# coqui-ai/TTS

Measured on NVIDIA H100. Metric: audio_samples_per_sec, higher is better.
Workload: dtype f32

## Files before the change

### tts_b200/csrc/common.cuh

```cuda
#pragma once
#include <cuda_runtime.h>
#include <stdint.h>
#include <stdio.h>
#include <atomic>
#include <mutex>
#include <string>
#include <vector>

namespace b200tts {

void set_error(const char* fmt, ...);
const char* last_error();

#define B200_CUDA_OK(expr)                                                                  \
    do {                                                                                    \
        cudaError_t _e = (expr);                                                            \
        if (_e != cudaSuccess) {                                                            \
            ::b200tts::set_error("%s:%d: %s -> %s", __FILE__, __LINE__, #expr,              \
                                 cudaGetErrorString(_e));                                   \
            return 2;                                                                       \
        }                                                                                   \
    } while (0)

#define B200_REQUIRE(cond, ...)                                                             \
// ... 53 lines not shown
};

struct ConvIO {
    const float* x = nullptr; long long x_bs = 0; int x_cs = 0; int Tin = 0;
    const float* xmask = nullptr; long long xmask_bs = 0;
    float in_slope = 1.0f;
    const float* cond = nullptr; long long cond_bs = 0;
    float* y = nullptr; long long y_bs = 0; int y_cs = 0; int Tout = 0;
    const float* res = nullptr; long long res_bs = 0; int res_cs = 0;
    const float* ymask = nullptr; long long ymask_bs = 0;
    float* y2 = nullptr; long long y2_bs = 0; int y2_cs = 0;
    int split = 0;
    float scale = 1.0f;
    float post_div = 1.0f;
    int act = ACT_NONE;
    float act_param = 0.f;
    int flags = 0;
    int B = 1;
    unsigned* peak_bits = nullptr;
    const int* lens = nullptr; int rate_out = 1, need_out = 0, rate_in = 1, need_in = 0;
    int q_lo = 0, q_hi = 0x7fffffff, in_lo = 0, in_hi = 0x7fffffff;
    int reflect = 0;
    int near_src = 0;
    const float* film = nullptr; long long film_bs = 0; int film_cs = 0; int film_half = 0;
    const float* act_add = nullptr;
};

int pack_conv(ConvLayer& L, const float* w, const float* bias, int Cout, int Cin, int K, int dil, int pad,
              int gate_half = 0, const int* in_perm = nullptr, const int* out_perm = nullptr);
int pack_conv_transpose(ConvLayer& L, const float* w, const float* bias, int Cin, int Cout, int Kt, int stride,
                        int padding, int output_padding = 0);
void free_conv(ConvLayer& L);
int launch_conv(const ConvLayer& L, const ConvIO& io, cudaStream_t stream);
int conv_tc_error_flag();
int pack_tc(void** dst, const std::vector<float>& Wl, int rows, int Cin, int K, int prec, int G, float** rscale = nullptr);
int tc_device(int** err, int* num_sms, size_t* max_smem);
enum : int { DISPATCH_FMA = 0, DISPATCH_TC3 = 3, DISPATCH_TC3_GROUPED = 5, DISPATCH_ROW1 = 6,
             DISPATCH_TC16 = 8, DISPATCH_TC16_GROUPED = 9,
             DISPATCH_ATTN_TC3 = 10, DISPATCH_ATTN_FMA = 11,
             DISPATCH_TC3W_TF32 = 12, DISPATCH_TC3W_F16X3 = 14, DISPATCH_FMA_WG = 16,
             DISPATCH_LSTM_BI = 18, DISPATCH_LSTM_CELL = 19, DISPATCH_HMM_LINEAR = 20, DISPATCH_HMM_STEP = 21,
             DISPATCH_PWGAN_TC = 22, DISPATCH_PWGAN_AUX = 23 };
void dispatch_begin();
int dispatch_end(int* ids, int cap);
void dispatch_note(int id);
inline int conv_transpose_out_len(const ConvLayer& L, int Tin) {
    return (Tin - 1) * L.ups - 2 * L.tr_pad + L.tr_kernel + L.tr_outpad;
}

template <class T> inline int upload(T** dst, const T* src, size_t n) {
    *dst = nullptr;
    if (n == 0) return 0;
    B200_CUDA_OK(cudaMalloc((void**)dst, n * sizeof(T)));
    B200_CUDA_OK(cudaMemcpy(*dst, src, n * sizeof(T), cudaMemcpyHostToDevice));
    return 0;
}

struct Arena {
    char* base; size_t cap; size_t off;
    Arena(void* p, size_t bytes) : base((char*)p), cap(bytes), off(0) {}
    float* f32(size_t n) {
        size_t bytes = (n * sizeof(float) + 255) & ~size_t(255);
        if (off + bytes > cap) return nullptr;
        float* r = (float*)(base + off);
        off += bytes;
        return r;
// ... 6 lines not shown
```

### tts_b200/csrc/conv1d.cu

```cuda
#include "common.cuh"
#include "engines.cuh"
#include "conv_tc.cuh"
#include "conv_tc3.cuh"

#include <cuda_bf16.h>
#include <cuda_fp16.h>
#include <stdarg.h>
#include <string.h>

#include <algorithm>
#include <cmath>

namespace b200tts {

static thread_local char g_err[1024] = "";
unsigned long long g_launch_count = 0;

void set_error(const char* fmt, ...) {
    va_list ap;
    va_start(ap, fmt);
    vsnprintf(g_err, sizeof(g_err), fmt, ap);
    va_end(ap);
}
const char* last_error() { return g_err; }
// ... 711 lines not shown
}
static void set_ragged(tc3::Tc3Args& t, const ConvKArgs& a, size_t& smem, size_t max_smem) {
    t.lens = nullptr; t.rate_q = 1; t.need_q = 0; t.rate_in = 1; t.need_in = 0; t.pref_off = 0;
    if (!a.lens) return;
    const size_t off = (smem + 15) / 16 * 16, extra = tc3::ragged_table_bytes(t.B);
    if (off + extra > max_smem) return;
    t.lens = a.lens; t.rate_q = a.rate_out; t.need_q = a.need_out; t.rate_in = a.rate_in; t.need_in = a.need_in;
    t.pref_off = (int)off;
    smem = off + extra;
}
static void set_window(tc3::Tc3Args& t, const ConvKArgs& a) {
    t.Tin = std::min(a.Tin, a.in_hi);
    t.q_lo = a.q_lo; t.q_hi = a.q_hi; t.in_lo = a.in_lo; t.t_lo = a.q_lo / t.tstep;
    const int hi = std::min(a.Tq, a.q_hi);
    t.n_ttiles = std::max(0, (hi + t.tstep - 1) / t.tstep - t.t_lo);
}

static int tc_device_init(int d) {
    int smem_optin = 0;
    B200_CUDA_OK(cudaDeviceGetAttribute(&smem_optin, cudaDevAttrMaxSharedMemoryPerBlockOptin, d));
    for (int p : {tc::PREC_FP32, tc::PREC_BF16, tc::PREC_FP16, tc::PREC_F16X3}) {
        for (bool lean : {true, false})
            B200_CUDA_OK(cudaFuncSetAttribute(tc3::plain_kernel(p, lean), cudaFuncAttributeMaxDynamicSharedMemorySize, smem_optin));
        B200_CUDA_OK(cudaFuncSetAttribute(tc3::plain_kernel(p, true, true), cudaFuncAttributeMaxDynamicSharedMemorySize, smem_optin));
        for (int g : {2, 4})
            for (bool refl : {false, true})
                B200_CUDA_OK(cudaFuncSetAttribute(tc3::grouped_kernel(g, p, refl), cudaFuncAttributeMaxDynamicSharedMemorySize,
                                                  smem_optin));
        for (bool near : {false, true})
            if (tc3::wavegrad_kernel(p, near))
                B200_CUDA_OK(cudaFuncSetAttribute(tc3::wavegrad_kernel(p, near), cudaFuncAttributeMaxDynamicSharedMemorySize,
                                                  smem_optin));
    }
    int* flag = nullptr;
    B200_CUDA_OK(cudaHostAlloc((void**)&flag, 2 * sizeof(int), cudaHostAllocMapped | cudaHostAllocPortable));
    flag[0] = flag[tc::ERR_RANGE] = 0;
    g_tc_dev[d].err = flag;
    g_tc_dev[d].max_smem = smem_optin;
    B200_CUDA_OK(cudaDeviceGetAttribute(&g_tc_dev[d].num_sms, cudaDevAttrMultiProcessorCount, d));
    return 0;
}

int tc_device(int** err, int* num_sms, size_t* max_smem) {
    int dev = 0;
    if (int rc = device_once(g_tc_once, &dev, tc_device_init)) return rc;
    int* const g_tc_err = g_tc_dev[dev].err;
    B200_REQUIRE(*reinterpret_cast<volatile int*>(g_tc_err) == 0,
                 "tensor-core conv: an earlier launch on device %d hit a pipeline timeout (its output is invalid)", dev);
    volatile int* const range_err = reinterpret_cast<volatile int*>(g_tc_err + tc::ERR_RANGE);
    if (*range_err) {
        *range_err = 0;
        B200_REQUIRE(false, "tensor-core conv: an earlier split-fp16 launch on device %d read an activation with |x| >= 65504, "
                            "outside fp16's range (its output is invalid; B200TTS_PRECISION_TF32X3 takes such models)", dev);
    }
    *err = g_tc_err;
    if (num_sms) *num_sms = g_tc_dev[dev].num_sms;
    if (max_smem) *max_smem = (size_t)g_tc_dev[dev].max_smem;
    return 0;
}

static int try_launch_tc(const ConvLayer& L, const ConvIO& io, const ConvKArgs& a, cudaStream_t st) {
    if (L.tc_prec == TC_NONE || a.Tq < 128) return -1;
    if (a.act == ACT_LOGCLAMP || a.act == ACT_TANH) return -1;
    if (!(a.in_slope >= 0.f && a.in_slope <= 1.f)) return -1;
    const bool needs_v3 = (a.flags & (EPI_MASK_PRE | EPI_SPLIT | EPI_ACCUM2 | EPI_GATE)) != 0;
    int* g_tc_err = nullptr;
// ... 25 lines not shown
    t.mask_pre = (a.flags & EPI_MASK_PRE) ? 1 : 0;
    t.gate = (a.flags & EPI_GATE) ? 1 : 0;
    t.split = (a.flags & EPI_SPLIT) ? a.split : 0;
    t.y2 = a.y2; t.y2_bs = a.y2_bs; t.y2_cs = a.y2_cs; t.accum2 = (a.flags & EPI_ACCUM2) ? 1 : 0;
    t.rows_pad = rows_pad; t.raw_w = rows_pad + 4;
    t.B = io.B; t.n_rtiles = (L.Rows + tc3::MROWS - 1) / tc3::MROWS;
    set_window(t, a);
    t.err = g_tc_err;
    size_t smem = tc3::smem_bytes3(rows_pad, L.tc_prec);
    set_ragged(t, a, smem, max_smem);
    const bool plain_epi = L.ups == 1 && !t.gate && t.split == 0 && !t.relu && !t.ymask && t.scale == 1.f && t.post_div == 1.f;
    const bool reflect = a.reflect != 0;
    if (reflect && !grouped && !plain_epi) return -1;
    if (wg) {
        t.near_src = a.near_src; t.near_scale = a.near_scale;
        t.film = a.film; t.film_bs = a.film_bs; t.film_cs = a.film_cs; t.film_half = a.film_half;
        t.act_add = a.act_add; t.lrelu = a.act == ACT_LRELU; t.act_param = a.act_param;
    }
    const tc3::Tc3Kernel k = wg ? tc3::wavegrad_kernel(L.tc_prec, a.near_src > 0)
                                : grouped ? tc3::grouped_kernel(G, L.tc_prec, reflect) : tc3::plain_kernel(L.tc_prec, plain_epi, reflect);
    const long long tiles = (long long)t.B * t.n_ttiles * t.n_rtiles;
    const int grid = (int)std::max(1LL, tiles < num_sms ? tiles : num_sms);
    B200_CUDA_OK(launch_tc3(k, grid, smem, st, t));
    count_launch();
    const bool b16 = L.tc_prec == tc::PREC_BF16 || L.tc_prec == tc::PREC_FP16;
    if (wg)
        dispatch_note((L.tc_prec == tc::PREC_F16X3 ? DISPATCH_TC3W_F16X3 : DISPATCH_TC3W_TF32) + (a.near_src > 0 ? 1 : 0));
    else
        dispatch_note(grouped ? (b16 ? DISPATCH_TC16_GROUPED : DISPATCH_TC3_GROUPED) : (b16 ? DISPATCH_TC16 : DISPATCH_TC3));
    B200_CUDA_OK(cudaGetLastError());
    return 0;
}

int conv_tc_error_flag() {
    int f = 0;
    for (int d = 0; d < MAX_DEVICES; ++d) {
        if (!g_tc_dev[d].err) continue;
        const volatile int* e = g_tc_dev[d].err;
        if (e[0]) f |= 1;
        if (e[tc::ERR_RANGE]) f |= 2;
    }
    return f;
}

int launch_conv(const ConvLayer& L, const ConvIO& io, cudaStream_t st) {
    B200_REQUIRE(L.w && io.x && io.y, "launch_conv: null tensor");
    ConvKArgs a;
    memset(&a, 0, sizeof(a));
    a.x = io.x; a.x_bs = io.x_bs; a.x_cs = io.x_cs; a.Tin = io.Tin;
    a.xmask = io.xmask; a.xmask_bs = io.xmask_bs; a.in_slope = io.in_slope;
    a.w = L.w; a.bias = L.bias; a.cond = io.cond; a.cond_bs = io.cond_bs;
    a.Cin = L.Cin; a.CinPad = L.CinPad; a.K = L.K; a.dil = L.dil; a.pad = L.pad; a.Rows = L.Rows; a.ups = L.ups;
    a.y = io.y; a.y_bs = io.y_bs; a.y_cs = io.y_cs; a.Tout = io.Tout;
    a.Tq = (L.ups > 1) ? (io.Tout + L.ups - 1) / L.ups : io.Tout;
    a.res = io.res; a.res_bs = io.res_bs; a.res_cs = io.res_cs;
    a.ymask = io.ymask; a.ymask_bs = io.ymask_bs;
    a.y2 = io.y2; a.y2_bs = io.y2_bs; a.y2_cs = io.y2_cs; a.split = io.split;
    a.scale = io.scale; a.post_div = io.post_div; a.act = io.act; a.act_param = io.act_param; a.flags = io.flags;
    a.lens = io.lens; a.rate_out = io.rate_out; a.need_out = io.need_out; a.rate_in = io.rate_in; a.need_in = io.need_in;
    a.q_lo = std::max(0, io.q_lo); a.q_hi = io.q_hi; a.in_lo = std::max(0, io.in_lo); a.in_hi = io.in_hi;
    const bool windowed = a.q_lo > 0 || a.q_hi < a.Tq;
    a.reflect = io.reflect ? 1 : 0;
    if (a.reflect) {
        B200_REQUIRE(L.pad <= io.Tin - 1, "launch_conv: reflection padding %d needs at least %d input columns, got %d", L.pad,
                     L.pad + 1, io.Tin);
        B200_REQUIRE(!io.lens && !windowed && a.in_lo == 0 && a.in_hi == 0x7fffffff && L.ups == 1 && !io.xmask,
// ... 67 lines not shown
```

### tts_b200/csrc/conv_tc3.cuh

```cuda
#pragma once
#include <cuda_runtime.h>
#include <stdint.h>

#include "conv_tc.cuh"

namespace b200tts {
namespace tc3 {

using namespace tc;

constexpr int TT2 = 256;
constexpr int MROWS = 128;
constexpr int KC2 = 8;
constexpr int KC16 = 16;
constexpr int RAWS = 324;
constexpr int NRAW = 3;
constexpr int NA2 = 2;
constexpr int NB2 = 3;
constexpr int ACC_LD = 260;
constexpr int ACC_BYTES = MROWS * ACC_LD * 4;
constexpr int NPW = 3;
constexpr int NPROD = 32 * NPW;
constexpr int NCONS = 256;
constexpr int W_PROD = 8, W_LOAD = 8 + NPW;
constexpr int NTHREADS2 = 32 * (W_LOAD + 1);

struct Tc3Args {
    const float* x; long long x_bs; int x_cs; int Tin;
    float in_slope;
    const void* w;
    const float* rscale;
    const float* bias;
    const float* cond; long long cond_bs;
    int Cin, K, dil, pad, Rows, N;
    float* y; long long y_bs; int y_cs; int Tout;
    int ups;
    int Tq;
    const float* res; long long res_bs; int res_cs;
    const float* ymask; long long ymask_bs;
    float scale; float post_div; int relu; int accum; int mask_post;
    int mask_pre;
    int gate;
    int split;
    float* y2; long long y2_bs; int y2_cs; int accum2;
    int KJ;
    int dil_blk;
    int tstep;
    int rows_pad;
    int raw_w;
    int B, n_ttiles, n_rtiles;
    int* err;
    const int* lens; int rate_q, need_q, rate_in, need_in;
    int pref_off;
    int q_lo, q_hi, in_lo, t_lo;
    int near_src; float near_scale;
    const float* film; long long film_bs; int film_cs, film_half;
    const float* act_add; int lrelu; float act_param;
};

__device__ __forceinline__ int near_col(int t, int src, int dst, float scale) {
    if (dst == src) return t;
    if (dst == 2 * src) return t >> 1;
    return min((int)floorf(__fmul_rn((float)t, scale)), src - 1);
}

static inline size_t smem_bytes3(int rows_pad, int prec = PREC_FP32) {
    const bool b16 = prec == PREC_BF16 || prec == PREC_FP16;
    const size_t raw_ch = b16 ? KC16 : KC2, nsl = b16 ? 2 : 4;
    return (size_t)NRAW * raw_ch * RAWS * 4 + (size_t)NA2 * (nsl * rows_pad * 16) + NB2 * (nsl * MROWS * 16) + ACC_BYTES + 512;
}
static inline size_t ragged_table_bytes(int B) { return ((size_t)(B + 1) * sizeof(int) + 15) / 16 * 16; }

__device__ __forceinline__ void cp_async16(uint32_t dst, const void* src) {
    asm volatile("cp.async.cg.shared.global [%0], [%1], 16;" ::"r"(dst), "l"(src) : "memory");
}
__device__ __forceinline__ void cp_async16_zfill(uint32_t dst, const void* src, uint32_t src_bytes) {
    asm volatile("cp.async.cg.shared.global [%0], [%1], 16, %2;" ::"r"(dst), "l"(src), "r"(src_bytes) : "memory");
}
__device__ __forceinline__ void cp_async4_zfill(uint32_t dst, const void* src, uint32_t src_bytes) {
    asm volatile("cp.async.ca.shared.global [%0], [%1], 4, %2;" ::"r"(dst), "l"(src), "r"(src_bytes) : "memory");
}
__device__ __forceinline__ void named_bar_sync(int id, int n) { asm volatile("bar.sync %0, %1;" ::"r"(id), "r"(n) : "memory"); }
__device__ __forceinline__ void acc_ld16(const float* p, float* v) {
#pragma unroll
    for (int j = 0; j < 4; ++j) {
        const float4 t = *reinterpret_cast<const float4*>(p + 4 * j);
        v[4 * j] = t.x; v[4 * j + 1] = t.y; v[4 * j + 2] = t.z; v[4 * j + 3] = t.w;
    }
}

constexpr int TSTEP_GROUPED = 240;

template <bool HR, bool HA, bool SC>
__device__ __forceinline__ void lean_tile(const float* at, const float* bias, const float* rscale, const float* cond, int lane,
                                          const float* rq, float* yq, long long rcs, long long ycs, int row0, int Rows,
                                          bool do_st) {
    const int r8 = lane & 7, p4 = lane >> 3;
    const float* rrow[4];
    float* yrow[4];
    bool st_ok[4];
    float bv[4], sv[4];
#pragma unroll
    for (int i = 0; i < 4; ++i) {
        const int ri = row0 + 8 * i + r8, rci = ri < Rows ? ri : Rows - 1;
        rrow[i] = rq + (long long)rci * rcs + 4 * p4;
        yrow[i] = yq + (long long)rci * ycs + 4 * p4;
        st_ok[i] = do_st && ri < Rows;
        bv[i] = bias[rci];
        if (cond) bv[i] += __ldg(cond + rci);
        sv[i] = SC ? rscale[rci] : 1.f;
    }
    const float* ap = at + r8 * ACC_LD + 4 * p4;
    float r0[16], r1[16];
    auto pf = [&](int cg, float* r_) {
        if constexpr (HR) {
#pragma unroll
            for (int i = 0; i < 4; ++i)
                asm volatile("ld.global.v4.f32 {%0,%1,%2,%3}, [%4];" : "=f"(r_[4 * i]), "=f"(r_[4 * i + 1]), "=f"(r_[4 * i + 2]), "=f"(r_[4 * i + 3]) : "l"(rrow[i] + cg));
        }
    };
    auto group = [&](int cg, const float* rv, float* rn) {
        float o[16];
        if (cg + 16 < 128) pf(cg + 16, rn);
        if constexpr (HA) {
// ... 192 lines not shown
        if (rok) prefetch(0, rA, oA);
#pragma unroll 1
        for (int cg = 0; cg < 128; cg += 32) {
            group(cg, rA, oA, rB, oB);
            group(cg + 16, rB, oB, rA, oA);
        }
    } else {
        if (!rok) return;
        const int co = rc / ups, ph = rc - co * ups;
        float* yrow = a.y + (long long)b * a.y_bs + (long long)co * a.y_cs + ph;
        for (int cg = 0; cg < 128; cg += 16) {
            float v[16];
            acc_ld(arow + cg, v);
#pragma unroll
            for (int i = 0; i < 16; ++i) {
                const int q = qb + cg + i;
                float u = v[i] + bias;
                if (a.relu) u = fmaxf(u, 0.f);
                const long long t = (long long)q * ups;
                if (q < a.Tq && t + ph < a.Tout) yrow[t] = u;
            }
        }
    }
}

template <bool SC>
__device__ __noinline__ void general_tile_call(const Tc3Args& a_ref, const float* arow, int b, int rt, int q0, int lq, int half,
                                               int lane) {
    const Tc3Args a = a_ref;
    general_tile_body<SC>(a, arow, b, rt, q0, lq, half, lane);
}

template <int GRP, bool SC>
__device__ __forceinline__ void grouped_tile(const Tc3Args& a, const float* accs, int b, int q0, int lq, int half, int lane) {
    constexpr int CH = 128 / GRP;
    constexpr int NQ = CH / 32;
    constexpr int NV = 4 * NQ;
    const int tq = lq * 32 + lane;
    const int co = (tq * NQ) >> 2;
    const int coff = 4 * ((tq & (4 / NQ - 1)) * NQ);
    const int cbeg = half ? 128 : 0;
    const int cend = half ? a.tstep : min(128, a.tstep);
    const bool has_res = a.res != nullptr, acc_r = a.accum != 0;
    const bool vec_ok = ((a.y_cs & 3) == 0) && ((a.y_bs & 3) == 0) && ((reinterpret_cast<uintptr_t>(a.y) & 15) == 0) &&
                        (!a.res || (((a.res_cs & 3) == 0) && ((a.res_bs & 3) == 0) && ((reinterpret_cast<uintptr_t>(a.res) & 15) == 0)));
    const bool fast = vec_ok && (q0 + a.tstep <= a.Tout);
    const float* rrow = has_res ? a.res + (long long)b * a.res_bs + (long long)co * a.res_cs : nullptr;
    float* yrow = a.y + (long long)b * a.y_bs + (long long)co * a.y_cs;
    float bias = a.bias[co];
    if (a.cond) bias += __ldg(a.cond + (long long)b * a.cond_bs + co);
    const float rs = SC ? a.rscale[co] : 1.f;
    auto load = [&](const float* rr, int q, float* dst) {
#pragma unroll
        for (int j = 0; j < NQ; ++j) {
            const int qq = q + 4 * j;
            if (fast || (vec_ok && qq + 3 < a.Tout)) {
                const float4 t = *reinterpret_cast<const float4*>(rr + qq);
                dst[4 * j] = t.x; dst[4 * j + 1] = t.y; dst[4 * j + 2] = t.z; dst[4 * j + 3] = t.w;
            } else {
#pragma unroll
                for (int e = 0; e < 4; ++e) dst[4 * j + e] = rr[min(qq + e, a.Tout - 1)];
            }
        }
    };
#pragma unroll 1
    for (int cg = cbeg; cg < cend; cg += 16) {
        float R[NV], rv[NV], ov[NV];
        if (has_res) load(rrow, q0 + cg + coff, rv);
        if (acc_r) load(yrow, q0 + cg + coff, ov);
        const float* p = accs + co * ACC_LD + cg + coff;
#pragma unroll
        for (int i = 0; i < NV; ++i) {
            const float p0 = p[i], p1 = p[CH * ACC_LD + a.dil + i];
            float s = p0 + p1;
            if constexpr (GRP == 4) s += p[2 * CH * ACC_LD + 2 * a.dil + i] + p[3 * CH * ACC_LD + 3 * a.dil + i];
            if constexpr (SC) s *= rs;
            R[i] = s;
        }
#pragma unroll
        for (int i = 0; i < NV; ++i) {
            float u = R[i] + bias;
            if (a.relu) u = fmaxf(u, 0.f);
            if (has_res) u += rv[i];
            u *= a.scale;
            if (acc_r) u += ov[i];
            if (a.post_div != 1.f) u = u / a.post_div;
            R[i] = u;
        }
        const int q = q0 + cg + coff;
#pragma unroll
        for (int j = 0; j < NQ; ++j) {
            const int qq = q + 4 * j;
            if (fast || (vec_ok && qq + 3 < a.Tout)) {
                *reinterpret_cast<float4*>(yrow + qq) = make_float4(R[4 * j], R[4 * j + 1], R[4 * j + 2], R[4 * j + 3]);
            } else {
#pragma unroll
                for (int e = 0; e < 4; ++e) if (qq + e < a.Tout) yrow[qq + e] = R[4 * j + e];
            }
        }
    }
}

template <int GRP, bool LEAN = true, int PREC = PREC_FP32, bool REFL = false, bool NEAR = false, bool WG = false>
__device__ __forceinline__ void tc3_body(const Tc3Args& a) {
    extern __shared__ __align__(128) unsigned char smem[];
    constexpr bool X3 = PREC == PREC_F16X3;
    constexpr bool B16 = PREC == PREC_BF16 || PREC == PREC_FP16;
    constexpr int KCH = PREC != PREC_FP32 ? KC16 : KC2;
    constexpr int RCH = B16 ? KC16 : KC2;
    constexpr int SPC = KCH / RCH;
    constexpr int NSL = B16 ? 2 : 4;
    constexpr int SLC = PREC != PREC_FP32 ? 8 : 4;
    constexpr int NB = NB2;
    constexpr bool SC = X3;
    const int tid = threadIdx.x, warp = tid >> 5, lane = tid & 31;
    const int ROWS = a.rows_pad, RAWW = a.raw_w, K = a.KJ;
    const uint32_t rawStage = (uint32_t)RCH * RAWS * 4;
    const uint32_t slabA = (uint32_t)ROWS * 16, stageA = NSL * slabA;
    const uint32_t slabB = (uint32_t)MROWS * 16, stageB = NSL * slabB;
    unsigned char* smRaw = smem;
    unsigned char* smA = smRaw + NRAW * rawStage;
    unsigned char* smB = smA + NA2 * stageA;
    float* accs = reinterpret_cast<float*>(smB + NB * stageB);
    uint64_t* bars = reinterpret_cast<uint64_t*>(reinterpret_cast<unsigned char*>(accs) + ACC_BYTES);
    const int A_FULL = 0, A_EMPTY = NA2, B_FULL = 2 * NA2, B_EMPTY = 2 * NA2 + NB;
    const uint32_t bar0 = smem_u32(bars);
    auto BAR = [&](int i) { return bar0 + 8u * (uint32_t)i; };

    const int nchunks = (a.Cin + KCH - 1) / KCH;
    const bool ragged = a.lens != nullptr;
    int* pref = reinterpret_cast<int*>(smem + a.pref_off);
    if (ragged) {
        for (int b = tid; b < a.B; b += NTHREADS2) {
            const long long e = (long long)a.lens[b] * a.rate_q + a.need_q;
            const int ext = (int)(e < (long long)a.Tq ? (e > 0 ? e : 0) : (long long)a.Tq);
            const int t_hi = (min(ext, a.q_hi) + a.tstep - 1) / a.tstep;
// ... 197 lines not shown
                    }
                    *reinterpret_cast<uint4*>(base + i_dst[e]) = make_uint4(p[0], p[1], p[2], p[3]);
                }
            } else {
#pragma unroll
                for (int e = 0; e < MAXI; ++e) {
                    if (i_raw[e] < 0) continue;
                    float4 hi, lo;
                    float* ph = &hi.x; float* pl = &lo.x;
#pragma unroll
                    for (int i = 0; i < 4; ++i) {
                        const float w_ = fmaxf(u[e][i], u[e][i] * slope);
                        const float h = __uint_as_float(__float_as_uint(w_) & 0xFFFFE000u);
                        ph[i] = h;
                        pl[i] = w_ - h;
                    }
                    *reinterpret_cast<float4*>(base + i_dst[e]) = hi;
                    *reinterpret_cast<float4*>(base + 2 * slabA + i_dst[e]) = lo;
                }
            }
            if (++tr_ring == NRAW) tr_ring = 0;
            if (++tr_h < SPC) continue;
            tr_h = 0;
            fence_async_smem();
            __syncwarp();
            if (lane == 0) mbar_arrive(BAR(A_FULL + as));
            if (++tr_c == nchunks) { tr_c = 0; ++tr_it; tr_new = true; }
            if (++as == NA2) { as = 0; pa_empty ^= 1u; }
        }
        asm volatile("cp.async.wait_group 0;" ::: "memory");
        if (X3 && amax >= F16X3_MAX && a.err) { *reinterpret_cast<volatile int*>(a.err + ERR_RANGE) = 1; __threadfence_system(); }
    } else if (warp == W_LOAD) {
        if (lane < NB) {
            const int total = nchunks * K;
            const long long all = (long long)my_tiles * total;
            const uint32_t full = BAR(B_FULL + lane), empty = BAR(B_EMPTY + lane);
            const uint32_t dst = smem_u32(smB + lane * stageB);
            int it = 0, j = lane;
            while (j >= total && it < my_tiles) { j -= total; ++it; }
            int cur_it = -1;
            const unsigned char* wsrc = nullptr;
            uint32_t par = 1;
            bool ok = true, first = true;
            for (long long gi = lane; gi < all && ok; gi += NB) {
                if (it != cur_it) {
                    int b_, rt, q0_;
                    decode(it, b_, rt, q0_);
                    wsrc = reinterpret_cast<const unsigned char*>(a.w) + (size_t)rt * total * stageB;
                    cur_it = it;
                }
                if (!first) { ok = mbar_wait(empty, par, a.err); if (!ok) break; }
                mbar_expect_tx(full, stageB);
                bulk_g2s(dst, wsrc + (size_t)j * stageB, stageB, full);
                first = false;
                par ^= 1u;
                j += NB;
                while (j >= total) { j -= total; ++it; }
            }
        }
        __syncwarp();
    } else if (warp < W_PROD) {
        const int wg = warp >> 2, lq = warp & 3, half = warp >> 2;
        const uint64_t wdesc0 = make_desc(smem_u32(smB) + (uint32_t)wg * 64 * 16, slabB);
        const uint64_t wlo_off = (uint64_t)((2 * slabB) >> 4), wslot = (uint64_t)(stageB >> 4);
        const uint32_t whi_lds = smem_u32(smB) + (uint32_t)(lane >> 4) * slabB + (uint32_t)(warp * 16 + (lane & 15)) * 16;
        const uint64_t xstep = (uint64_t)a.dil_blk;
        bool ok = true;
        int sa = 0; uint32_t pa = 0;
        int sb = 0; uint32_t pb = 0;
        float* const st_row = accs + (wg * 64 + lq * 16 + (lane >> 2)) * ACC_LD + 2 * (lane & 3);
#pragma unroll 1
        for (int it = 0; it < my_tiles; ++it) {
            float d[128];
#pragma unroll
            for (int i = 0; i < 128; ++i) d[i] = 0.f;
            uint32_t acc = 0u;
            int rel_b = -1, rel_a = -1;
            auto release = [&]() {
                __syncwarp();
                if (lane == 0) {
                    if (rel_b >= 0) mbar_arrive(BAR(B_EMPTY + rel_b));
                    if (rel_a >= 0) mbar_arrive(BAR(A_EMPTY + rel_a));
                }
            };
#pragma unroll 1
            for (int c = 0; c < nchunks; ++c) {
// ... 10 lines not shown
                            ldsm_x4(whs, whi_lds + (uint32_t)sb * stageB);
#pragma unroll
                            for (int i = 0; i < 4; ++i) whs[i] = f16x2_times_2m11(whs[i]);
                        }
                        wgmma_fence();
                        if constexpr (PREC == PREC_BF16) {
                            wgmma_bf16_m64n256(d, w_hi, xh, acc);
                        } else if constexpr (PREC == PREC_FP16) {
                            wgmma_f16_m64n256(d, w_hi, xh, acc);
                        } else if constexpr (X3) {
                            wgmma_f16_m64n256_rs(d, whs, xl, acc);
                            wgmma_commit();
                            wgmma_f16_m64n256(d, w_lo, xh, 1u);
                            wgmma_f16_m64n256(d, w_hi, xh, 1u);
                        } else {
                            wgmma_tf32_m64n256(d, w_hi, xl, acc);
                            wgmma_tf32_m64n256(d, w_lo, xh, 1u);
                            wgmma_tf32_m64n256(d, w_hi, xh, 1u);
                        }
                        wgmma_commit();
                    }
                    wgmma_wait<1>();
                    release();
                    rel_b = sb;
                    rel_a = (k == K - 1) ? sa : -1;
                    acc = 1u;
                    xh += xstep; xl += xstep;
                    if (++sb == NB) { sb = 0; pb ^= 1u; }
                }
                if (++sa == NA2) { sa = 0; pa ^= 1u; }
            }
            wgmma_wait<0>();
            release();
            named_bar_sync(4, NCONS);
#pragma unroll
            for (int j = 0; j < 32; ++j) {
                *reinterpret_cast<float2*>(st_row + 8 * j) = make_float2(d[4 * j], d[4 * j + 1]);
                *reinterpret_cast<float2*>(st_row + 8 * ACC_LD + 8 * j) = make_float2(d[4 * j + 2], d[4 * j + 3]);
            }
            named_bar_sync(4, NCONS);
            if (!ok) continue;
            int b, rt, q0;
            decode(it, b, rt, q0);
            if constexpr (GRP > 1) {
                grouped_tile<GRP, SC>(a, accs, b, q0, lq, half, lane);
            } else {
                const int qb = q0 + half * 128;
                const float* at = accs + lq * 32 * ACC_LD + half * 128;
                const bool lean = LEAN && a.ups == 1 && !a.gate && a.split == 0 && !a.relu && !a.ymask && a.scale == 1.f &&
                                  a.post_div == 1.f && qb + 128 <= a.Tout &&
                                  ((a.y_cs & 3) == 0) && ((a.y_bs & 3) == 0) && ((reinterpret_cast<uintptr_t>(a.y) & 15) == 0) &&
                                  (!a.res || (((a.res_cs & 3) == 0) && ((a.res_bs & 3) == 0) && ((reinterpret_cast<uintptr_t>(a.res) & 15) == 0)));
                if (lean) {
                    const int row0 = rt * MROWS + lq * 32;
                    const float* cond = a.cond ? a.cond + (long long)b * a.cond_bs : nullptr;
                    float* yq = a.y + (long long)b * a.y_bs + qb;
                    const bool hres = a.res != nullptr, hacc = a.accum != 0;
                    const float* rq = hres ? a.res + (long long)b * a.res_bs + qb : yq;
                    if (hres) { if (hacc) lean_tile<true, true, SC>(at, a.bias, a.rscale, cond, lane, rq, yq, a.res_cs, a.y_cs, row0, a.Rows, true);
                                else lean_tile<true, false, SC>(at, a.bias, a.rscale, cond, lane, rq, yq, a.res_cs, a.y_cs, row0, a.Rows, true); }
                    else { if (hacc) lean_tile<false, true, SC>(at, a.bias, a.rscale, cond, lane, rq, yq, 0, a.y_cs, row0, a.Rows, true);
                           else lean_tile<false, false, SC>(at, a.bias, a.rscale, cond, lane, rq, yq, 0, a.y_cs, row0, a.Rows, true); }
                } else if constexpr (LEAN) {
                    general_tile_call<SC>(a, at + lane * ACC_LD, b, rt, q0, lq, half, lane);
                } else {
                    general_tile_body<SC, WG>(a, at + lane * ACC_LD, b, rt, q0, lq, half, lane);
                }
            }
        }
    }
}

template <int PREC, bool REFL = false>
__global__ void __launch_bounds__(NTHREADS2, 1) conv1d_tc3_kernel(const __grid_constant__ Tc3Args a) { tc3_body<1, true, PREC, REFL>(a); }
template <int PREC>
__global__ void __launch_bounds__(NTHREADS2, 1) conv1d_tc3x_kernel(const __grid_constant__ Tc3Args a) { tc3_body<1, false, PREC>(a); }
template <int GRP, int PREC, bool REFL = false>
__global__ void __launch_bounds__(NTHREADS2, 1) conv1d_tc3g_kernel(const __grid_constant__ Tc3Args a) { tc3_body<GRP, true, PREC, REFL>(a); }

template <int PREC, bool NEAR>
__global__ void __launch_bounds__(NTHREADS2, 1) conv1d_tc3w_kernel(const __grid_constant__ Tc3Args a) {
    tc3_body<1, false, PREC, false, NEAR, true>(a);
}

typedef void (*Tc3Kernel)(const Tc3Args);
static inline Tc3Kernel wavegrad_kernel(int prec, bool near) {
    if (prec == PREC_F16X3) return near ? conv1d_tc3w_kernel<PREC_F16X3, true> : conv1d_tc3w_kernel<PREC_F16X3, false>;
    if (prec == PREC_FP32) return near ? conv1d_tc3w_kernel<PREC_FP32, true> : conv1d_tc3w_kernel<PREC_FP32, false>;
    return nullptr;
}
static inline Tc3Kernel plain_kernel(int prec, bool lean, bool reflect = false) {
    if (reflect) {
        if (prec == PREC_BF16) return conv1d_tc3_kernel<PREC_BF16, true>;
        if (prec == PREC_FP16) return conv1d_tc3_kernel<PREC_FP16, true>;
        if (prec == PREC_F16X3) return conv1d_tc3_kernel<PREC_F16X3, true>;
        return conv1d_tc3_kernel<PREC_FP32, true>;
    }
    if (prec == PREC_BF16) return lean ? conv1d_tc3_kernel<PREC_BF16> : conv1d_tc3x_kernel<PREC_BF16>;
    if (prec == PREC_FP16) return lean ? conv1d_tc3_kernel<PREC_FP16> : conv1d_tc3x_kernel<PREC_FP16>;
    if (prec == PREC_F16X3) return lean ? conv1d_tc3_kernel<PREC_F16X3> : conv1d_tc3x_kernel<PREC_F16X3>;
    return lean ? conv1d_tc3_kernel<PREC_FP32> : conv1d_tc3x_kernel<PREC_FP32>;
}
template <bool REFL>
static inline Tc3Kernel grouped_kernel_t(int grp, int prec) {
    if (prec == PREC_BF16) return grp == 2 ? conv1d_tc3g_kernel<2, PREC_BF16, REFL> : conv1d_tc3g_kernel<4, PREC_BF16, REFL>;
    if (prec == PREC_FP16) return grp == 2 ? conv1d_tc3g_kernel<2, PREC_FP16, REFL> : conv1d_tc3g_kernel<4, PREC_FP16, REFL>;
    if (prec == PREC_F16X3) return grp == 2 ? conv1d_tc3g_kernel<2, PREC_F16X3, REFL> : conv1d_tc3g_kernel<4, PREC_F16X3, REFL>;
    return grp == 2 ? conv1d_tc3g_kernel<2, PREC_FP32, REFL> : conv1d_tc3g_kernel<4, PREC_FP32, REFL>;
}
static inline Tc3Kernel grouped_kernel(int grp, int prec = PREC_FP32, bool reflect = false) {
    return reflect ? grouped_kernel_t<true>(grp, prec) : grouped_kernel_t<false>(grp, prec);
// ... 5 lines not shown
```

### tts_b200/csrc/engines.cuh

```cuda
#pragma once
#include <algorithm>
#include <string.h>

#include "../../include/tts_b200.h"
#include "common.cuh"

namespace b200tts {

struct Hifigan {
    b200tts_hifigan_config c;
    ConvLayer conv_pre, cond, conv_post;
    std::vector<ConvLayer> ups;
    std::vector<std::vector<ConvLayer>> rb_c1, rb_c2;
    int prec = B200TTS_PRECISION_FP32;
    ~Hifigan();
    int init(const b200tts_hifigan_config& cfg, const float* const* w, int nw, int precision = B200TTS_PRECISION_FP32);
    void stage_dims(int T, std::vector<int>& C, std::vector<int>& L) const;
    size_t workspace_bytes(int B, int T) const;
    int out_len(int T) const;
    int forward(const float* x, const float* g, int B, int T, float* wav, void* ws, size_t ws_bytes,
                cudaStream_t st, unsigned* peak_bits = nullptr, const int* lens = nullptr, int frame_begin = 0,
                int frame_end = -1) const;
    int need_P = 0;
    std::vector<int> need_OUT, need_U, need_q_ups, rate;
    std::vector<std::vector<int>> need_T1, need_X;
    void plan_margins();
};

struct WaveNet {
    int H = 0, K = 0, L = 0, cond_ch = 0;
    ConvLayer cond;
    std::vector<ConvLayer> in_layers, res_skip;
    ~WaveNet();
    int init(int hidden, int kernel_size, int dilation_rate, int num_layers, int cond_channels,
             const float* const* w, int* consumed);
    size_t scratch_floats(int B, int T) const;
    int forward(float* h, float* out, const float* mask, const float* g, int B, int T, float* acts, float* condv,
                cudaStream_t st, const int* lens = nullptr) const;
};

struct Flow {
    struct Block { ConvLayer pre, post; WaveNet wn; bool odd = false; };
    b200tts_flow_config c;
    bool fwd = false;
    std::vector<Block*> blocks;
    ~Flow();
    int init(const b200tts_flow_config& cfg, const float* const* w, int nw, int forward_direction = 0);
// ... 311 lines not shown
```

### tts_b200/csrc/hifigan.cu

```cuda
#include "engines.cuh"

namespace b200tts {

Hifigan::~Hifigan() {
    free_conv(conv_pre);
    free_conv(cond);
    free_conv(conv_post);
    for (auto& l : ups) free_conv(l);
    for (auto& v : rb_c1) for (auto& l : v) free_conv(l);
    for (auto& v : rb_c2) for (auto& l : v) free_conv(l);
}

int Hifigan::init(const b200tts_hifigan_config& cfg, const float* const* w, int nw, int precision) {
    c = cfg;
    B200_REQUIRE(precision == B200TTS_PRECISION_FP32 || precision == B200TTS_PRECISION_BF16 ||
                     precision == B200TTS_PRECISION_FP16 || precision == B200TTS_PRECISION_TF32X3 ||
                     precision == B200TTS_PRECISION_F16X3,
                 "hifigan: unknown precision %d", precision);
    prec = precision;
    const int lp = precision == B200TTS_PRECISION_FP32     ? B200TTS_PRECISION_F16X3
                   : precision == B200TTS_PRECISION_TF32X3 ? B200TTS_PRECISION_FP32
                                                           : precision;
    B200_REQUIRE(c.num_upsamples >= 1 && c.num_upsamples <= 8 && c.num_kernels >= 1 && c.num_kernels <= 8 &&
                     c.num_dilations >= 1 && c.num_dilations <= 8,
                 "hifigan: unsupported config");
    const int type1 = (c.resblock_type == 1);
    const int expect = 2 + (c.cond_channels > 0 ? 2 : 0) + 2 * c.num_upsamples +
                       c.num_upsamples * c.num_kernels * c.num_dilations * (type1 ? 4 : 2) + 2;
    B200_REQUIRE(nw == expect, "hifigan: expected %d weight tensors, got %d", expect, nw);
    int i = 0;
    conv_pre.tc_prec = lp;
    int rc = pack_conv(conv_pre, w[i], w[i + 1], c.upsample_initial_channel, c.in_channels, 7, 1, 3);
    if (rc) return rc;
    i += 2;
    if (c.cond_channels > 0) {
        rc = pack_conv(cond, w[i], w[i + 1], c.upsample_initial_channel, c.cond_channels, 1, 1, 0);
        if (rc) return rc;
        i += 2;
    }
    ups.resize(c.num_upsamples);
    rb_c1.assign(c.num_upsamples * c.num_kernels, std::vector<ConvLayer>());
    rb_c2.assign(c.num_upsamples * c.num_kernels, std::vector<ConvLayer>());
    int ch = c.upsample_initial_channel;
    for (int s = 0; s < c.num_upsamples; ++s) {
        const int u = c.upsample_factors[s], k = c.upsample_kernel_sizes[s];
        ups[s].tc_prec = lp;
        rc = pack_conv_transpose(ups[s], w[i], w[i + 1], ch, ch / 2, k, u, (k - u) / 2);
// ... 162 lines not shown
        ConvIO io;
        io.x = xin0; io.x_bs = (long long)c.in_channels * x_pitch; io.x_cs = x_pitch; io.Tin = T;
        io.y = P; io.y_bs = (long long)C0 * Tp; io.y_cs = Tp; io.Tout = T; io.B = B;
        if (has_cond) { io.cond = condv; io.cond_bs = cond.RowsPad; }
        io.lens = lens; io.rate_out = 1; io.need_out = need_P; io.rate_in = 1; io.need_in = T;
        window(io);
        if ((rc = launch_conv(conv_pre, io, st))) return rc;
    }
    const float* cur = P;
    int curC = C0, curL = T, curPitch = Tp;
    const bool type1 = c.resblock_type == 1;
    for (int s = 0; s < c.num_upsamples; ++s) {
        const int Cs = C[s], Ls = L[s];
        const long long bs = (long long)Cs * Ls;
        {
            ConvIO io;
            io.x = cur; io.x_bs = (long long)curC * curPitch; io.x_cs = curPitch; io.Tin = curL; io.in_slope = 0.1f;
            io.y = U; io.y_bs = bs; io.y_cs = Ls; io.Tout = Ls; io.B = B;
            io.lens = lens; io.rate_in = (s == 0) ? 1 : rate[s - 1]; io.need_in = (s == 0) ? need_P : need_OUT[s - 1];
            io.rate_out = io.rate_in; io.need_out = need_q_ups[s];
            window(io);
            if ((rc = launch_conv(ups[s], io, st))) return rc;
        }
        for (int j = 0; j < c.num_kernels; ++j) {
            const auto& c1 = rb_c1[s * c.num_kernels + j];
            const auto& c2 = rb_c2[s * c.num_kernels + j];
            const float* xin = U;
            int need_xin = need_U[s];
            float* pp[2] = {R, T1};
            for (int n = 0; n < c.num_dilations; ++n) {
                const bool last = (n == c.num_dilations - 1);
                const float* convin = xin;
                const ConvLayer* lastconv = &c1[n];
                if (type1) {
                    ConvIO io;
                    io.x = xin; io.x_bs = bs; io.x_cs = Ls; io.Tin = Ls; io.in_slope = 0.1f;
                    io.y = T1; io.y_bs = bs; io.y_cs = Ls; io.Tout = Ls; io.B = B;
                    io.lens = lens; io.rate_in = io.rate_out = rate[s];
                    io.need_in = need_xin; io.need_out = need_T1[s * c.num_kernels + j][n];
                    window(io);
                    if ((rc = launch_conv(c1[n], io, st))) return rc;
                    convin = T1;
                    lastconv = &c2[n];
                }
                ConvIO io;
                io.x = convin; io.x_bs = bs; io.x_cs = Ls; io.Tin = Ls; io.in_slope = 0.1f;
                io.res = xin; io.res_bs = bs; io.res_cs = Ls;
                io.B = B; io.Tout = Ls; io.y_bs = bs; io.y_cs = Ls;
                float* dst;
                if (last) {
                    dst = OUT;
                    if (j > 0) io.flags |= EPI_ACCUM;
                    if (j == c.num_kernels - 1) io.post_div = (float)c.num_kernels;
                } else {
                    dst = type1 ? R : pp[n & 1];
                }
                io.y = dst;
                io.lens = lens; io.rate_in = io.rate_out = rate[s];
                io.need_in = type1 ? need_T1[s * c.num_kernels + j][n] : need_xin;
                io.need_out = need_X[s * c.num_kernels + j][n];
                window(io);
                if ((rc = launch_conv(*lastconv, io, st))) return rc;
                xin = dst;
                need_xin = io.need_out;
            }
        }
        cur = OUT;
        curC = Cs;
        curL = Ls;
        curPitch = Ls;
    }
    {
        ConvIO io;
        io.x = cur; io.x_bs = (long long)curC * curPitch; io.x_cs = curPitch; io.Tin = curL; io.in_slope = 0.01f;
        io.y = wav; io.y_bs = (long long)c.out_channels * curL; io.y_cs = curL; io.Tout = curL; io.B = B;
        io.act = ACT_TANH;
        io.peak_bits = peak_bits;
        io.lens = lens; io.rate_in = io.rate_out = rate.empty() ? 1 : rate.back(); io.need_in = need_OUT.empty() ? 0 : need_OUT.back();
        io.need_out = 0;
        window(io);
        if (lens) {
            B200_REQUIRE(B <= 65535, "hifigan_forward: batch too large");
            const int lo = io.q_lo, hi = std::min(io.q_hi, curL);
            const dim3 grid((unsigned)std::max(1, std::min((hi - lo + 255) / 256, 64)), (unsigned)B);
            zero_past_end_kernel<<<grid, 256, 0, st>>>(wav, c.out_channels, curL, lens, io.rate_out, lo, hi);
            count_launch();
            B200_CUDA_OK(cudaGetLastError());
        }
        if ((rc = launch_conv(conv_post, io, st))) return rc;
    }
    return 0;
}

}
```

Before: 30.66 million.

## Fuse HiFi-GAN type-1 resblock conv pairs into one tensor-core kernel

Adds a paired grouped TC3 kernel that runs the first conv of a type-1 resblock, applies bias and leaky ReLU, writes the intermediate tile as split f16 into shared memory, and then runs the second conv from it. The intermediate no longer round-trips through global memory and one launch per pair is saved. The cost is recomputing halo columns for each time tile (a smaller tstep) and extra register and shared-memory pressure. The fused path applies only to F16X3 grouped layers that pass alignment and shape checks; anything else falls back to two launches.

Result: faster. 32.02 million (median of 6 runs) (+4.4%).

```diff
diff --git a/tts_b200/csrc/common.cuh b/tts_b200/csrc/common.cuh
--- a/tts_b200/csrc/common.cuh
+++ b/tts_b200/csrc/common.cuh
@@ -109,6 +109,7 @@
                         int padding, int output_padding = 0);
 void free_conv(ConvLayer& L);
 int launch_conv(const ConvLayer& L, const ConvIO& io, cudaStream_t stream);
+int launch_conv_pair(const ConvLayer& c1, const ConvLayer& c2, const ConvIO& io1, const ConvIO& io2, cudaStream_t stream);
 int conv_tc_error_flag();
 int pack_tc(void** dst, const std::vector<float>& Wl, int rows, int Cin, int K, int prec, int G, float** rscale = nullptr);
 int tc_device(int** err, int* num_sms, size_t* max_smem);
diff --git a/tts_b200/csrc/conv1d.cu b/tts_b200/csrc/conv1d.cu
--- a/tts_b200/csrc/conv1d.cu
+++ b/tts_b200/csrc/conv1d.cu
@@ -767,6 +767,8 @@
                 B200_CUDA_OK(cudaFuncSetAttribute(tc3::wavegrad_kernel(p, near), cudaFuncAttributeMaxDynamicSharedMemorySize,
                                                   smem_optin));
     }
+    for (tc3::Tc3Kernel k : {tc3::conv1d_tc3p_kernel<2>, tc3::conv1d_tc3p_kernel<4>})
+        B200_CUDA_OK(cudaFuncSetAttribute(k, cudaFuncAttributeMaxDynamicSharedMemorySize, smem_optin));
     int* flag = nullptr;
     B200_CUDA_OK(cudaHostAlloc((void**)&flag, 2 * sizeof(int), cudaHostAllocMapped | cudaHostAllocPortable));
     flag[0] = flag[tc::ERR_RANGE] = 0;
@@ -858,6 +860,64 @@
     return 0;
 }
 
+int launch_conv_pair(const ConvLayer& c1, const ConvLayer& c2, const ConvIO& io1, const ConvIO& io2, cudaStream_t st) {
+    const int G = c1.tc_grp, C = c1.Rows;
+    if (c1.tc_prec != tc::PREC_F16X3 || c2.tc_prec != tc::PREC_F16X3 || G == 0 || c2.tc_grp != G) return -1;
+    if (c1.ups != 1 || c2.ups != 1 || c1.Cin != C || c2.Cin != C || c2.Rows != C) return -1;
+    auto plain = [](const ConvIO& io) {
+        return !io.xmask && !io.cond && !io.ymask && !io.y2 && !io.peak_bits && io.act == ACT_NONE && io.scale == 1.f &&
+               !io.reflect && io.near_src == 0 && !io.film && !io.act_add && io.in_slope >= 0.f && io.in_slope <= 1.f;
+    };
+    auto aligned = [](const void* p, long long bs, int cs) { return (reinterpret_cast<uintptr_t>(p) & 15) == 0 && bs % 4 == 0 && cs % 4 == 0; };
+    if (!plain(io1) || !plain(io2) || io1.flags != 0 || io1.res || io1.post_div != 1.f) return -1;
+    if ((io2.flags & ~EPI_ACCUM) != 0 || io2.x != io1.y || io2.res != io1.x || io2.lens != io1.lens || io2.B != io1.B) return -1;
+    if (io2.y == io1.x) return -1;
+    const int L = io2.Tout;
+    if (io1.Tin != L || io1.Tout != L || io2.Tin != L || L < tc3::TT2) return -1;
+    if (!aligned(io1.x, io1.x_bs, io1.x_cs) || !aligned(io1.y, io1.y_bs, io1.y_cs)) return -1;
+    if ((G - 1) * c1.dil > 15 || (G - 1) * c2.dil > 15) return -1;
+    int* g_tc_err = nullptr;
+    int num_sms = 0;
+    size_t max_smem = 0;
+    if (int rc = tc_device(&g_tc_err, &num_sms, &max_smem)) return rc;
+    const int J1 = (c1.K + G - 1) / G, J2 = (c2.K + G - 1) / G;
+    const int rp1 = (tc3::TT2 + (J1 - 1) * G * c1.dil + 7) / 8 * 8, rp2 = (tc3::TT2 + (J2 - 1) * G * c2.dil + 7) / 8 * 8;
+    if (rp1 > 320 || tc3::smem_bytes3(rp1, tc::PREC_F16X3) > max_smem || rp2 > tc3::T1_ROWS_MAX) return -1;
+    const int valid1 = tc3::TT2 - (G - 1) * c1.dil;
+    const int tstep = std::min(tc3::TSTEP_GROUPED, (valid1 - (c2.K - 1) * c2.dil) / 16 * 16);
+    if (tstep < 16) return -1;
+    ConvKArgs a;
+    memset(&a, 0, sizeof(a));
+    a.Tin = io1.Tin; a.Tq = L;
+    a.q_lo = std::max(0, io2.q_lo); a.q_hi = io2.q_hi; a.in_lo = std::max(0, io1.in_lo); a.in_hi = io1.in_hi;
+    a.lens = io1.lens; a.rate_out = io2.rate_out; a.need_out = io2.need_out; a.rate_in = io1.rate_in; a.need_in = io1.need_in;
+    tc3::Tc3Args t;
+    memset(&t, 0, sizeof(t));
+    t.x = io1.x; t.x_bs = io1.x_bs; t.x_cs = io1.x_cs; t.in_slope = io1.in_slope;
+    t.w = c1.w_tcg; t.rscale = c1.tc_rscale; t.bias = c1.bias;
+    t.Cin = C; t.K = c1.K; t.dil = c1.dil; t.pad = c1.pad + c2.pad; t.Rows = C; t.N = tc3::MROWS;
+    t.KJ = J1; t.dil_blk = G * c1.dil; t.tstep = tstep; t.rows_pad = rp1; t.raw_w = rp1 + 4;
+    t.y = io2.y; t.y_bs = io2.y_bs; t.y_cs = io2.y_cs; t.Tout = L; t.ups = 1; t.Tq = L;
+    t.res = io2.res; t.res_bs = io2.res_bs; t.res_cs = io2.res_cs;
+    t.scale = 1.f; t.post_div = io2.post_div; t.accum = (io2.flags & EPI_ACCUM) ? 1 : 0;
+    t.w2 = c2.w_tcg; t.rscale2 = c2.tc_rscale; t.bias2 = c2.bias;
+    t.KJ2 = J2; t.dil2 = c2.dil; t.dil_blk2 = G * c2.dil; t.rows_pad2 = rp2; t.pad2 = c2.pad; t.t1_slope = io2.in_slope;
+    t.B = io1.B; t.n_rtiles = 1;
+    set_window(t, a);
+    t.err = g_tc_err;
+    size_t smem = tc3::smem_bytes3(rp1, tc::PREC_F16X3);
+    set_ragged(t, a, smem, max_smem);
+    const tc3::Tc3Kernel k = G == 2 ? tc3::conv1d_tc3p_kernel<2> : tc3::conv1d_tc3p_kernel<4>;
+    const long long tiles = (long long)t.B * t.n_ttiles;
+    const int grid = (int)std::max(1LL, tiles < num_sms ? tiles : num_sms);
+    B200_CUDA_OK(launch_tc3(k, grid, smem, st, t));
+    count_launch();
+    dispatch_note(DISPATCH_TC3_GROUPED);
+    dispatch_note(DISPATCH_TC3_GROUPED);
+    B200_CUDA_OK(cudaGetLastError());
+    return 0;
+}
+
 int conv_tc_error_flag() {
     int f = 0;
     for (int d = 0; d < MAX_DEVICES; ++d) {
diff --git a/tts_b200/csrc/conv_tc3.cuh b/tts_b200/csrc/conv_tc3.cuh
--- a/tts_b200/csrc/conv_tc3.cuh
+++ b/tts_b200/csrc/conv_tc3.cuh
@@ -56,6 +56,8 @@
     int near_src; float near_scale;
     const float* film; long long film_bs; int film_cs, film_half;
     const float* act_add; int lrelu; float act_param;
+    const void* w2; const float* rscale2; const float* bias2;
+    int KJ2, dil2, dil_blk2, rows_pad2, pad2; float t1_slope;
 };
 
 __device__ __forceinline__ int near_col(int t, int src, int dst, float scale) {
@@ -90,6 +92,7 @@
 }
 
 constexpr int TSTEP_GROUPED = 240;
+constexpr int T1_ROWS_MAX = 272;
 
 template <bool HR, bool HA, bool SC>
 __device__ __forceinline__ void lean_tile(const float* at, const float* bias, const float* rscale, const float* cond, int lane,
@@ -348,7 +351,8 @@
 }
 
 template <int GRP, bool SC>
-__device__ __forceinline__ void grouped_tile(const Tc3Args& a, const float* accs, int b, int q0, int lq, int half, int lane) {
+__device__ __forceinline__ void grouped_tile(const Tc3Args& a, const float* accs, int b, int q0, int lq, int half, int lane,
+                                             const float* bias_p, const float* rscale_p, int dil) {
     constexpr int CH = 128 / GRP;
     constexpr int NQ = CH / 32;
     constexpr int NV = 4 * NQ;
@@ -363,9 +367,9 @@
     const bool fast = vec_ok && (q0 + a.tstep <= a.Tout);
     const float* rrow = has_res ? a.res + (long long)b * a.res_bs + (long long)co * a.res_cs : nullptr;
     float* yrow = a.y + (long long)b * a.y_bs + (long long)co * a.y_cs;
-    float bias = a.bias[co];
+    float bias = bias_p[co];
     if (a.cond) bias += __ldg(a.cond + (long long)b * a.cond_bs + co);
-    const float rs = SC ? a.rscale[co] : 1.f;
+    const float rs = SC ? rscale_p[co] : 1.f;
     auto load = [&](const float* rr, int q, float* dst) {
 #pragma unroll
         for (int j = 0; j < NQ; ++j) {
@@ -387,9 +391,9 @@
         const float* p = accs + co * ACC_LD + cg + coff;
 #pragma unroll
         for (int i = 0; i < NV; ++i) {
-            const float p0 = p[i], p1 = p[CH * ACC_LD + a.dil + i];
+            const float p0 = p[i], p1 = p[CH * ACC_LD + dil + i];
             float s = p0 + p1;
-            if constexpr (GRP == 4) s += p[2 * CH * ACC_LD + 2 * a.dil + i] + p[3 * CH * ACC_LD + 3 * a.dil + i];
+            if constexpr (GRP == 4) s += p[2 * CH * ACC_LD + 2 * dil + i] + p[3 * CH * ACC_LD + 3 * dil + i];
             if constexpr (SC) s *= rs;
             R[i] = s;
         }
@@ -417,7 +421,8 @@
     }
 }
 
-template <int GRP, bool LEAN = true, int PREC = PREC_FP32, bool REFL = false, bool NEAR = false, bool WG = false>
+template <int GRP, bool LEAN = true, int PREC = PREC_FP32, bool REFL = false, bool NEAR = false, bool WG = false,
+          bool PAIR = false>
 __device__ __forceinline__ void tc3_body(const Tc3Args& a) {
     extern __shared__ __align__(128) unsigned char smem[];
     constexpr bool X3 = PREC == PREC_F16X3;
@@ -681,7 +686,7 @@
         if (X3 && amax >= F16X3_MAX && a.err) { *reinterpret_cast<volatile int*>(a.err + ERR_RANGE) = 1; __threadfence_system(); }
     } else if (warp == W_LOAD) {
         if (lane < NB) {
-            const int total = nchunks * K;
+            const int total1 = nchunks * K, total = PAIR ? total1 + nchunks * a.KJ2 : total1;
             const long long all = (long long)my_tiles * total;
             const uint32_t full = BAR(B_FULL + lane), empty = BAR(B_EMPTY + lane);
             const uint32_t dst = smem_u32(smB + lane * stageB);
@@ -689,18 +694,20 @@
             while (j >= total && it < my_tiles) { j -= total; ++it; }
             int cur_it = -1;
             const unsigned char* wsrc = nullptr;
+            const unsigned char* const wsrc2 =
+                PAIR ? reinterpret_cast<const unsigned char*>(a.w2) - (size_t)total1 * stageB : nullptr;
             uint32_t par = 1;
             bool ok = true, first = true;
             for (long long gi = lane; gi < all && ok; gi += NB) {
                 if (it != cur_it) {
                     int b_, rt, q0_;
                     decode(it, b_, rt, q0_);
-                    wsrc = reinterpret_cast<const unsigned char*>(a.w) + (size_t)rt * total * stageB;
+                    wsrc = reinterpret_cast<const unsigned char*>(a.w) + (size_t)rt * total1 * stageB;
                     cur_it = it;
                 }
                 if (!first) { ok = mbar_wait(empty, par, a.err); if (!ok) break; }
                 mbar_expect_tx(full, stageB);
-                bulk_g2s(dst, wsrc + (size_t)j * stageB, stageB, full);
+                bulk_g2s(dst, (!PAIR || j < total1 ? wsrc : wsrc2) + (size_t)j * stageB, stageB, full);
                 first = false;
                 par ^= 1u;
                 j += NB;
@@ -777,18 +784,107 @@
             }
             wgmma_wait<0>();
             release();
-            named_bar_sync(4, NCONS);
-#pragma unroll
-            for (int j = 0; j < 32; ++j) {
-                *reinterpret_cast<float2*>(st_row + 8 * j) = make_float2(d[4 * j], d[4 * j + 1]);
-                *reinterpret_cast<float2*>(st_row + 8 * ACC_LD + 8 * j) = make_float2(d[4 * j + 2], d[4 * j + 3]);
-            }
-            named_bar_sync(4, NCONS);
+            auto store_acc = [&]() {
+                named_bar_sync(4, NCONS);
+#pragma unroll
+                for (int j = 0; j < 32; ++j) {
+                    *reinterpret_cast<float2*>(st_row + 8 * j) = make_float2(d[4 * j], d[4 * j + 1]);
+                    *reinterpret_cast<float2*>(st_row + 8 * ACC_LD + 8 * j) = make_float2(d[4 * j + 2], d[4 * j + 3]);
+                }
+                named_bar_sync(4, NCONS);
+            };
+            store_acc();
+            if constexpr (PAIR) {
+                constexpr int CH = 128 / GRP, NG8 = CH / 8;
+                constexpr int MAXT = (T1_ROWS_MAX * NG8 + NCONS - 1) / NCONS;
+                int b, rt, q0;
+                decode(it, b, rt, q0);
+                const int R2 = a.rows_pad2, n_t1 = R2 * NG8, dil1 = a.dil;
+                const int valid1 = TT2 - (GRP - 1) * dil1, t1c0 = q0 - a.pad2;
+                const float slope2 = a.t1_slope;
+                float t1max = 0.f;
+                uint32_t th[MAXT][4], tl[MAXT][4];
+#pragma unroll
+                for (int e = 0; e < MAXT; ++e) {
+                    const int idx = tid + e * NCONS, g8 = idx / R2, r = idx - g8 * R2, col = t1c0 + r;
+#pragma unroll
+                    for (int i = 0; i < 4; ++i) { th[e][i] = 0u; tl[e][i] = 0u; }
+                    if (ok && idx < n_t1 && r < valid1 && col >= 0 && col < a.Tout) {
+                        float w[8];
+#pragma unroll
+                        for (int j = 0; j < 8; ++j) {
+                            const int c = g8 * 8 + j;
+                            const float* p = accs + c * ACC_LD + r;
+                            float s = p[0] + p[CH * ACC_LD + dil1];
+                            if constexpr (GRP == 4) s += p[2 * CH * ACC_LD + 2 * dil1] + p[3 * CH * ACC_LD + 3 * dil1];
+                            s *= a.rscale[c];
+                            const float u = s + a.bias[c];
+                            w[j] = fmaxf(u, u * slope2);
+                            t1max = fmaxf(t1max, fabsf(w[j]));
+                        }
+#pragma unroll
+                        for (int i = 0; i < 4; ++i) split_f16x2(w[2 * i], w[2 * i + 1], th[e][i], tl[e][i]);
+                    }
+                }
+                if (t1max >= F16X3_MAX && a.err) { *reinterpret_cast<volatile int*>(a.err + ERR_RANGE) = 1; __threadfence_system(); }
+                named_bar_sync(4, NCONS);
+                unsigned char* const t1 = reinterpret_cast<unsigned char*>(accs);
+                const uint32_t slabT = (uint32_t)R2 * 16, stageT = 4 * slabT;
+#pragma unroll
+                for (int e = 0; e < MAXT; ++e) {
+                    const int idx = tid + e * NCONS, g8 = idx / R2, r = idx - g8 * R2;
+                    if (idx >= n_t1) continue;
+                    unsigned char* dst = t1 + (g8 >> 1) * stageT + (g8 & 1) * slabT + r * 16;
+                    *reinterpret_cast<uint4*>(dst) = make_uint4(th[e][0], th[e][1], th[e][2], th[e][3]);
+                    *reinterpret_cast<uint4*>(dst + 2 * slabT) = make_uint4(tl[e][0], tl[e][1], tl[e][2], tl[e][3]);
+                }
+                fence_async_smem();
+                named_bar_sync(4, NCONS);
+#pragma unroll
+                for (int i = 0; i < 128; ++i) d[i] = 0.f;
+                acc = 0u;
+                rel_b = rel_a = -1;
+                const uint32_t t1u = smem_u32(t1);
+                const uint64_t xstep2 = (uint64_t)a.dil_blk2;
+#pragma unroll 1
+                for (int c = 0; c < nchunks; ++c) {
+                    uint64_t xh = make_desc(t1u + c * stageT, slabT), xl = make_desc(t1u + c * stageT + 2 * slabT, slabT);
+#pragma unroll 1
+                    for (int k = 0; k < a.KJ2; ++k) {
+                        if (ok) ok = mbar_wait(BAR(B_FULL + sb), pb, a.err);
+                        if (ok) {
+                            const uint64_t w_hi = wdesc0 + (uint64_t)sb * wslot, w_lo = w_hi + wlo_off;
+                            uint32_t whs[4];
+                            ldsm_x4(whs, whi_lds + (uint32_t)sb * stageB);
+#pragma unroll
+                            for (int i = 0; i < 4; ++i) whs[i] = f16x2_times_2m11(whs[i]);
+                            wgmma_fence();
+                            wgmma_f16_m64n256_rs(d, whs, xl, acc);
+                            wgmma_commit();
+                            wgmma_f16_m64n256(d, w_lo, xh, 1u);
+                            wgmma_f16_m64n256(d, w_hi, xh, 1u);
+                            wgmma_commit();
+                        }
+                        wgmma_wait<1>();
+                        release();
+                        rel_b = sb;
+                        acc = 1u;
+                        xh += xstep2; xl += xstep2;
+                        if (++sb == NB) { sb = 0; pb ^= 1u; }
+                    }
+                }
+                wgmma_wait<0>();
+                release();
+                store_acc();
+                if (!ok) continue;
+                grouped_tile<GRP, SC>(a, accs, b, q0, lq, half, lane, a.bias2, a.rscale2, a.dil2);
+                continue;
+            }
             if (!ok) continue;
             int b, rt, q0;
             decode(it, b, rt, q0);
             if constexpr (GRP > 1) {
-                grouped_tile<GRP, SC>(a, accs, b, q0, lq, half, lane);
+                grouped_tile<GRP, SC>(a, accs, b, q0, lq, half, lane, a.bias, a.rscale, a.dil);
             } else {
                 const int qb = q0 + half * 128;
                 const float* at = accs + lq * 32 * ACC_LD + half * 128;
@@ -822,6 +918,11 @@
 __global__ void __launch_bounds__(NTHREADS2, 1) conv1d_tc3x_kernel(const __grid_constant__ Tc3Args a) { tc3_body<1, false, PREC>(a); }
 template <int GRP, int PREC, bool REFL = false>
 __global__ void __launch_bounds__(NTHREADS2, 1) conv1d_tc3g_kernel(const __grid_constant__ Tc3Args a) { tc3_body<GRP, true, PREC, REFL>(a); }
+template <int GRP>
+__global__ void __launch_bounds__(NTHREADS2, 1) conv1d_tc3p_kernel(const __grid_constant__ Tc3Args a) {
+    static_assert(MROWS / GRP / KC16 * 4 * T1_ROWS_MAX * 16 <= ACC_BYTES, "T1 must fit in the accumulator tile");
+    tc3_body<GRP, true, PREC_F16X3, false, false, false, true>(a);
+}
 
 template <int PREC, bool NEAR>
 __global__ void __launch_bounds__(NTHREADS2, 1) conv1d_tc3w_kernel(const __grid_constant__ Tc3Args a) {
diff --git a/tts_b200/csrc/engines.cuh b/tts_b200/csrc/engines.cuh
--- a/tts_b200/csrc/engines.cuh
+++ b/tts_b200/csrc/engines.cuh
@@ -13,6 +13,7 @@
     std::vector<ConvLayer> ups;
     std::vector<std::vector<ConvLayer>> rb_c1, rb_c2;
     int prec = B200TTS_PRECISION_FP32;
+    bool fuse_pairs = true;
     ~Hifigan();
     int init(const b200tts_hifigan_config& cfg, const float* const* w, int nw, int precision = B200TTS_PRECISION_FP32);
     void stage_dims(int T, std::vector<int>& C, std::vector<int>& L) const;
diff --git a/tts_b200/csrc/hifigan.cu b/tts_b200/csrc/hifigan.cu
--- a/tts_b200/csrc/hifigan.cu
+++ b/tts_b200/csrc/hifigan.cu
@@ -13,6 +13,8 @@
 
 int Hifigan::init(const b200tts_hifigan_config& cfg, const float* const* w, int nw, int precision) {
     c = cfg;
+    const char* unfused = getenv("B200TTS_UNFUSED_RESBLOCK");
+    fuse_pairs = !(unfused && *unfused && strcmp(unfused, "0") != 0);
     B200_REQUIRE(precision == B200TTS_PRECISION_FP32 || precision == B200TTS_PRECISION_BF16 ||
                      precision == B200TTS_PRECISION_FP16 || precision == B200TTS_PRECISION_TF32X3 ||
                      precision == B200TTS_PRECISION_F16X3,
@@ -241,15 +243,15 @@
                 const bool last = (n == c.num_dilations - 1);
                 const float* convin = xin;
                 const ConvLayer* lastconv = &c1[n];
+                float* const t1buf = xin == T1 ? R : T1;
+                ConvIO io1;
                 if (type1) {
-                    ConvIO io;
-                    io.x = xin; io.x_bs = bs; io.x_cs = Ls; io.Tin = Ls; io.in_slope = 0.1f;
-                    io.y = T1; io.y_bs = bs; io.y_cs = Ls; io.Tout = Ls; io.B = B;
-                    io.lens = lens; io.rate_in = io.rate_out = rate[s];
-                    io.need_in = need_xin; io.need_out = need_T1[s * c.num_kernels + j][n];
-                    window(io);
-                    if ((rc = launch_conv(c1[n], io, st))) return rc;
-                    convin = T1;
+                    io1.x = xin; io1.x_bs = bs; io1.x_cs = Ls; io1.Tin = Ls; io1.in_slope = 0.1f;
+                    io1.y = t1buf; io1.y_bs = bs; io1.y_cs = Ls; io1.Tout = Ls; io1.B = B;
+                    io1.lens = lens; io1.rate_in = io1.rate_out = rate[s];
+                    io1.need_in = need_xin; io1.need_out = need_T1[s * c.num_kernels + j][n];
+                    window(io1);
+                    convin = t1buf;
                     lastconv = &c2[n];
                 }
                 ConvIO io;
@@ -262,14 +264,24 @@
                     if (j > 0) io.flags |= EPI_ACCUM;
                     if (j == c.num_kernels - 1) io.post_div = (float)c.num_kernels;
                 } else {
-                    dst = type1 ? R : pp[n & 1];
+                    dst = type1 ? (xin == T1 ? T1 : R) : pp[n & 1];
                 }
                 io.y = dst;
                 io.lens = lens; io.rate_in = io.rate_out = rate[s];
                 io.need_in = type1 ? need_T1[s * c.num_kernels + j][n] : need_xin;
                 io.need_out = need_X[s * c.num_kernels + j][n];
                 window(io);
-                if ((rc = launch_conv(*lastconv, io, st))) return rc;
+                rc = -1;
+                if (type1 && fuse_pairs) {
+                    io.y = dst == xin ? (xin == R ? T1 : R) : dst;
+                    if ((rc = launch_conv_pair(c1[n], c2[n], io1, io, st)) == 0) dst = io.y;
+                    io.y = dst;
+                }
+                if (rc == -1) {
+                    if (type1 && (rc = launch_conv(c1[n], io1, st))) return rc;
+                    rc = launch_conv(*lastconv, io, st);
+                }
+                if (rc) return rc;
                 xin = dst;
                 need_xin = io.need_out;
             }
```
